# SamsungLabs/Metis

Measured on AMD Instinct MI355X. Metric: best_plan_iter_time_ms, lower is better.
Workload: dtype bf16; 1 GPU; model=gpt3-2.7b, global_batch=16, seq_len=2048, parallelism=dp1_tp1_pp1, microbatch=16

## Files before the change

### metis_amd/models/gpt.py

```python

from __future__ import annotations

import math
from dataclasses import dataclass
from typing import List, Optional

import torch
import torch.utils.checkpoint
import torch.distributed as dist
import torch.nn as nn
import torch.nn.functional as F

from metis_amd.ops import LayerNorm
from metis_amd.ops import residual as _res
from metis_amd.ops.attention import decode_attention, packed_flash_attention
from metis_amd.ops.cross_entropy import cross_entropy
from metis_amd.ops.mlp import fused_mlp
from metis_amd.ops.relayout import heads_merge, qkv_split_transpose
from metis_amd.partial_grads import mark_partial

import os as _os


@dataclass(frozen=True)
class GPTModelSpec:
    name: str
    hidden_size: int
    num_layers: int
    num_heads: int
    vocab_size: int
    seq_length: int
    ffn_hidden_size: Optional[int] = None
    num_kv_heads: Optional[int] = None

    @property
    def ffn(self) -> int:
        return self.ffn_hidden_size or 4 * self.hidden_size

    @property
# ... 193 lines not shown
        return _VocabParallelCrossEntropyBF16.apply(
            logits2d.contiguous(), labels, group)
    return _VocabParallelCrossEntropy.apply(
        logits2d.float().contiguous(), labels, group)


def _init_linear(weight: torch.Tensor, fan_in: int) -> None:
    std = 1.0 / math.sqrt(fan_in)
    nn.init.normal_(weight, mean=0.0, std=std)


class ColumnParallelLinear(nn.Module):

    def __init__(self, in_features: int, out_features: int, tp: int, dtype):
        super().__init__()
        assert out_features % tp == 0
        self.out_per_rank = out_features // tp
        self.weight = nn.Parameter(torch.empty(self.out_per_rank, in_features, dtype=dtype))
        self.bias = nn.Parameter(torch.zeros(self.out_per_rank, dtype=dtype))
        _init_linear(self.weight, in_features)

    def forward(self, x: torch.Tensor, tp_group) -> torch.Tensor:
        x = _CopyToTP.apply(x, tp_group)
        return F.linear(x, self.weight, self.bias)


class RowParallelLinear(nn.Module):

    def __init__(self, in_features: int, out_features: int, tp: int, dtype):
        super().__init__()
        assert in_features % tp == 0
        self.in_per_rank = in_features // tp
        self.weight = nn.Parameter(torch.empty(out_features, self.in_per_rank, dtype=dtype))
        self.bias = nn.Parameter(torch.zeros(out_features, dtype=dtype))
        _init_linear(self.weight, in_features)

    def forward(self, x: torch.Tensor, tp_group) -> torch.Tensor:
        y = F.linear(x, self.weight)
        y = _ReduceFromTP.apply(y, tp_group)
        return y + self.bias


class GPTBlock(nn.Module):
    def __init__(self, spec: GPTModelSpec, tp: int, dtype):
        super().__init__()
        h = spec.hidden_size
        assert spec.num_heads % tp == 0, "num_heads must divide by tp"
        self.heads_per_rank = spec.num_heads // tp
        self.head_dim = spec.head_dim

        self.ln_attn = LayerNorm(h)
        self.qkv = ColumnParallelLinear(h, 3 * h, tp, dtype)
        self.proj = RowParallelLinear(h, h, tp, dtype)
        self.ln_mlp = LayerNorm(h)
        self.fc1 = ColumnParallelLinear(h, spec.ffn, tp, dtype)
        self.fc2 = RowParallelLinear(spec.ffn, h, tp, dtype)
        self._lt_mlp = _os.environ.get("METIS_FC1_EPILOGUE") == "1"


    def _cached_attention(self, q, k, v, mask=None):
        new, total = q.size(2), k.size(2)
        if mask is not None:
            return F.scaled_dot_product_attention(q, k, v, attn_mask=mask)
        if new == 1:
            return decode_attention(q, k, v)
        mask = torch.ones(new, total, dtype=torch.bool, device=q.device)
        mask = torch.tril(mask, diagonal=total - new)
        return F.scaled_dot_product_attention(q, k, v, attn_mask=mask)

    def _forward_fused(self, x: torch.Tensor, tp_group) -> torch.Tensor:
        x, y = _res.norm_passthrough(
            x, self.ln_attn.weight, self.ln_attn.bias, self.ln_attn.eps)
        qkv = self.qkv(y, tp_group)
        attn = packed_flash_attention(
            qkv, self.heads_per_rank, self.heads_per_rank, self.head_dim
        )
        part = _ReduceFromTP.apply(F.linear(attn, self.proj.weight), tp_group)
        x, y = _res.bias_residual_layer_norm(
            part, self.proj.bias, x, self.ln_mlp.weight, self.ln_mlp.bias,
            self.ln_mlp.eps)
        h = F.linear(_CopyToTP.apply(y, tp_group), self.fc1.weight,
                     self.fc1.bias.detach())
        a = _res.gelu_bgrad(h, self.fc1.bias)
        part = _ReduceFromTP.apply(F.linear(a, self.fc2.weight), tp_group)
        return _res.bias_residual_add(part, self.fc2.bias, x)

    def forward(self, x: torch.Tensor, tp_group, sp: bool = False,
                cache=None, layer_idx: int = 0) -> torch.Tensor:
        if cache is not None:
            residual = x
            y = self.ln_attn(x)
            qkv = self.qkv(y, tp_group)
            q, k, v = qkv_split_transpose(
                qkv, self.heads_per_rank, self.heads_per_rank, self.head_dim)
            k, v = cache.append(layer_idx, k, v)
            if hasattr(cache, "kv_lens") and q.size(2) == 1:
                scales = getattr(cache, "kv_scales", None)
                scales = scales(layer_idx) if scales is not None else None
                if scales is None:
                    attn = decode_attention(q, k, v, kv_lens=cache.kv_lens())
                else:
                    attn = decode_attention(q, k, v, kv_lens=cache.kv_lens(),
                                            k_scale=scales[0],
                                            v_scale=scales[1])
            else:
                am = getattr(cache, "attention_mask", None)
                mask = am(k.size(2), q.device) if am is not None else None
# ... 177 lines not shown
```

### metis_amd/ops/adamw.py

```python

from __future__ import annotations

from typing import Iterable, List, Optional

import torch
import torch.distributed as dist

from metis_amd import ops as _ops


class FusedAdamW:
    def __init__(
        self,
        params: Iterable[torch.nn.Parameter],
        lr: float = 1e-4,
        betas=(0.9, 0.95),
        eps: float = 1e-8,
        weight_decay: float = 0.1,
        shard_group: Optional[object] = None,
    ) -> None:
        self.params: List[torch.nn.Parameter] = [p for p in params if p.requires_grad]
        if not self.params:
            raise ValueError("no trainable parameters")
        self.lr = lr
        self.beta1, self.beta2 = betas
        self.eps = eps
        self.weight_decay = weight_decay
        self.step_count = 0
        self.shard_group = shard_group
        ws = dist.get_world_size(shard_group) if shard_group is not None else 1
        self._shard_ws = ws
# ... 69 lines not shown
            self.m.mul_(self.beta1).add_(g, alpha=1 - self.beta1)
            self.v.mul_(self.beta2).addcmul_(g, g, value=1 - self.beta2)
            mhat = self.m / (1 - self.beta1 ** self.step_count)
            vhat = self.v / (1 - self.beta2 ** self.step_count)
            self.master.add_(
                -self.lr * (mhat / (vhat.sqrt() + self.eps)
                            + self.weight_decay * self.master)
            )

    def _gather_weight_shards(self) -> torch.Tensor:
        full = torch.empty(self._n, dtype=torch.float32,
                           device=self.master.device)
        try:
            dist.all_gather_into_tensor(full, self.master, group=self.shard_group)
        except (RuntimeError, ValueError):
            parts = [torch.empty_like(self.master) for _ in range(self._shard_ws)]
            dist.all_gather(parts, self.master, group=self.shard_group)
            full = torch.cat(parts)
        return full

    @torch.no_grad()
    def step(self, grad_scale: float = 1.0, pre_gathered: bool = False) -> None:
        self.step_count += 1
        grads = self._grad_flat if pre_gathered else self._gather_grads()

        if self._shard_ws > 1:
            off, n = self._shard_off, self._shard_n
            model = (self._model_flat[off:off + n]
                     if self._model_flat is not None else torch.Tensor())
            self._update(grads[off:off + n], model, grad_scale)
            if self._model_flat is not None:
                shard = self._model_flat[off:off + n].clone()
                dist.all_gather_into_tensor(self._model_flat, shard,
                                            group=self.shard_group)
                return
            full = self._gather_weight_shards()
            for p, (o, pn) in zip(self.params, self._slices):
                p.copy_(full[o:o + pn].view_as(p).to(p.dtype))
            return

        model = self._model_flat if self._model_flat is not None else torch.Tensor()
        self._update(grads, model, grad_scale)
        if self._model_flat is not None:
            return
        for p, (off, n) in zip(self.params, self._slices):
            p.copy_(self.master[off:off + n].view_as(p).to(p.dtype))

    def state_dict(self) -> dict:
        return {
            "step": self.step_count,
            "master": self.master,
            "m": self.m,
            "v": self.v,
        }

    def load_state_dict(self, state: dict) -> None:
        self.step_count = state["step"]
        self.master.copy_(state["master"])
        self.m.copy_(state["m"])
        self.v.copy_(state["v"])
```

### metis_amd/ops/hip/bindings.cpp

```cpp
#include <torch/extension.h>

#include <vector>

std::vector<torch::Tensor> layernorm_fwd(
    torch::Tensor x, torch::Tensor gamma, torch::Tensor beta, double eps);
std::vector<torch::Tensor> layernorm_bwd(
    torch::Tensor dy, torch::Tensor x, torch::Tensor gamma,
    torch::Tensor mean, torch::Tensor rstd);
std::vector<torch::Tensor> bias_residual_layernorm_fwd(
    torch::Tensor y, torch::Tensor bias, torch::Tensor residual,
    torch::Tensor gamma, torch::Tensor beta, double eps);
torch::Tensor bias_residual_add(
    torch::Tensor y, torch::Tensor bias, torch::Tensor residual);
std::vector<torch::Tensor> layernorm_bwd_add(
    torch::Tensor dy, torch::Tensor dres, torch::Tensor x, torch::Tensor gamma,
    torch::Tensor mean, torch::Tensor rstd, bool want_colsum);
std::vector<torch::Tensor> gelu_tanh_bwd_bgrad(torch::Tensor h, torch::Tensor da);
void adamw_step(
    torch::Tensor master, torch::Tensor model, torch::Tensor grad,
    torch::Tensor m, torch::Tensor v,
    double lr, double beta1, double beta2, double eps,
    double weight_decay, long step, double grad_scale);
torch::Tensor attn_decode(
    torch::Tensor q, torch::Tensor k, torch::Tensor v, double scale);
// ... 46 lines not shown
torch::Tensor mfma_tile_probe(torch::Tensor a, torch::Tensor b);
torch::Tensor gemm8_bf16(torch::Tensor x, torch::Tensor w);
std::vector<torch::Tensor> rmsnorm_fwd(
    torch::Tensor x, torch::Tensor gamma, double eps);
std::vector<torch::Tensor> rmsnorm_bwd(
    torch::Tensor dy, torch::Tensor x, torch::Tensor gamma, torch::Tensor rstd);
torch::Tensor rope_apply(
    torch::Tensor x, torch::Tensor cos_t, torch::Tensor sin_t, bool backward);
torch::Tensor swiglu_fwd(torch::Tensor a, torch::Tensor b);
std::vector<torch::Tensor> swiglu_bwd(
    torch::Tensor dy, torch::Tensor a, torch::Tensor b);
std::vector<torch::Tensor> cross_entropy_fwd(
    torch::Tensor logits, torch::Tensor labels);
torch::Tensor cross_entropy_bwd(
    torch::Tensor logits, torch::Tensor labels, torch::Tensor lse,
    torch::Tensor grad_scale);
std::vector<torch::Tensor> qkv_split_transpose(
    torch::Tensor qkv, long nq, long nkv, long head_dim);
torch::Tensor qkv_split_transpose_bwd(
    torch::Tensor dq, torch::Tensor dk, torch::Tensor dv, long head_dim);
torch::Tensor heads_merge(torch::Tensor x);
torch::Tensor heads_unmerge(torch::Tensor y, long H);
torch::Tensor tr16_probe(long stride_elems);

PYBIND11_MODULE(TORCH_EXTENSION_NAME, m) {
    m.def("layernorm_fwd", &layernorm_fwd,
          "fused LayerNorm forward (bf16, fp32 stats)");
    m.def("layernorm_bwd", &layernorm_bwd,
          "fused LayerNorm backward (dx + dgamma/dbeta)");
    m.def("bias_residual_layernorm_fwd", &bias_residual_layernorm_fwd,
          "x = residual + (y + bias) with both bf16 roundings, then "
          "LayerNorm(x) -> (x, z, mean, rstd)");
    m.def("bias_residual_add", &bias_residual_add,
          "x = residual + (y + bias) with both bf16 roundings");
    m.def("layernorm_bwd_add", &layernorm_bwd_add,
          "LayerNorm backward with a residual gradient folded in -> "
          "(g = dres + dx, dgamma, dbeta, colsum of g in fp32 or empty)");
    m.def("gelu_tanh_bwd_bgrad", &gelu_tanh_bwd_bgrad,
          "tanh-GeLU backward -> (dh bf16, dbias = column sums of dh, fp32)");
    m.def("adamw_step", &adamw_step, "fused AdamW step");
    m.def("attn_fwd", &attn_fwd,
          "flash attention forward (causal, GQA) -> (O, LSE)");
    m.def("attn_bwd", &attn_bwd,
          "flash attention backward -> (dQ, dK_per_head, dV_per_head)");
    m.def("attn_bwd_delta", &attn_bwd_delta,
          "rowsum(dO * O) in fp32 -> [B,H,S] (contiguous bf16 inputs)");
// ... 49 lines not shown
          pybind11::arg("v_scale"), pybind11::arg("slots"),
          pybind11::arg("pos"));
    m.def("w8_linear", &w8_linear,
          "fp8 (e4m3fn) weight-only linear for 1 <= M <= 16 bf16 rows: "
          "scale[n] * (x @ w8^T) + bias, fp32 accumulation, split-K",
          pybind11::arg("x"), pybind11::arg("w8"), pybind11::arg("scale"),
          pybind11::arg("bias") = pybind11::none(),
          pybind11::arg("num_splits") = 0);
    m.def("w8_linear_auto_splits", &w8_linear_auto_splits,
          "split count w8_linear picks for num_splits = 0 (from N and K only)");
    m.def("ce_row_max", &ce_row_max, "per-row max of bf16 logits (fp32)");
    m.def("ce_row_sumexp", &ce_row_sumexp,
          "per-row sum(exp(x - m)) of bf16 logits (fp32)");
    m.def("qkv_rope_split", &qkv_rope_split,
          "fused QKV relayout + RoPE (neox) forward");
    m.def("qkv_rope_split_bwd", &qkv_rope_split_bwd,
          "fused QKV relayout + RoPE backward gather");
    m.def("lt_fp8_matmul", &lt_fp8_matmul,
          "fp8 e4m3 GEMM with per-tensor scales, bf16 out");
    m.def("lt_fc1_forward", &lt_fc1_forward,
          "hipblaslt GEMM with GELU_AUX_BIAS epilogue (fc1 fused)");
    m.def("lt_matmul_dgelu_bgrad", &lt_matmul_dgelu_bgrad,
          "hipblaslt GEMM with DGELU_BGRAD epilogue (fc2 data grad fused)");
    m.def("tr16_probe", &tr16_probe,
          "ds_read_b64_tr_b16 lane-semantics probe (debug)");
}
```

### metis_amd/ops/hip/lt_gemm.cpp

```cpp

#include <torch/extension.h>

#include <hipblaslt/hipblaslt.h>

#include <c10/hip/HIPStream.h>

#include <mutex>
#include <stdexcept>
#include <string>
#include <unordered_map>

namespace {

#define LT_CHECK(expr)                                                        \
    do {                                                                      \
        hipblasStatus_t s_ = (expr);                                          \
        TORCH_CHECK(s_ == HIPBLAS_STATUS_SUCCESS, "hipblaslt error ",         \
                    (int)s_, " at ", #expr);                                  \
    } while (0)

hipblasLtHandle_t lt_handle() {
    static hipblasLtHandle_t handle = [] {
        hipblasLtHandle_t h;
        LT_CHECK(hipblasLtCreate(&h));
        return h;
    }();
    return handle;
}

constexpr size_t kWorkspaceBytes = 64ull << 20;

torch::Tensor workspace(const torch::TensorOptions& opt) {
    static torch::Tensor ws;
    if (!ws.defined() || ws.numel() < (long)kWorkspaceBytes)
        ws = torch::empty({(long)kWorkspaceBytes},
                          opt.dtype(torch::kUInt8));
    return ws;
}

struct LtPlan {
    hipblasLtMatmulDesc_t desc{};
    hipblasLtMatrixLayout_t a{}, b{}, d{};
    hipblasLtMatmulAlgo_t algo{};
    bool has_algo = false;
};

std::unordered_map<std::string, LtPlan>& plan_cache() {
    static std::unordered_map<std::string, LtPlan> cache;
    return cache;
}
std::mutex cache_mutex;

LtPlan& get_plan(hipblasLtEpilogue_t epi, bool transa, long M, long N, long K,
                 const void* bias, const void* aux, long aux_ld) {
    std::lock_guard<std::mutex> lock(cache_mutex);
    std::string key = std::to_string((int)epi) + (transa ? "t" : "n") + "_" +
                      std::to_string(M) + "_" + std::to_string(N) + "_" +
                      std::to_string(K);
    auto it = plan_cache().find(key);
    if (it != plan_cache().end()) return it->second;

    LtPlan plan;
    LT_CHECK(hipblasLtMatmulDescCreate(&plan.desc, HIPBLAS_COMPUTE_32F,
                                       HIP_R_32F));
    hipblasOperation_t opA = transa ? HIPBLAS_OP_T : HIPBLAS_OP_N;
    hipblasOperation_t opN = HIPBLAS_OP_N;
    LT_CHECK(hipblasLtMatmulDescSetAttribute(
        plan.desc, HIPBLASLT_MATMUL_DESC_TRANSA, &opA, sizeof(opA)));
    LT_CHECK(hipblasLtMatmulDescSetAttribute(
        plan.desc, HIPBLASLT_MATMUL_DESC_TRANSB, &opN, sizeof(opN)));
    LT_CHECK(hipblasLtMatmulDescSetAttribute(
        plan.desc, HIPBLASLT_MATMUL_DESC_EPILOGUE, &epi, sizeof(epi)));
    if (bias != nullptr)
        LT_CHECK(hipblasLtMatmulDescSetAttribute(
            plan.desc, HIPBLASLT_MATMUL_DESC_BIAS_POINTER, &bias,
            sizeof(bias)));
    if (aux != nullptr) {
        LT_CHECK(hipblasLtMatmulDescSetAttribute(
            plan.desc, HIPBLASLT_MATMUL_DESC_EPILOGUE_AUX_POINTER, &aux,
            sizeof(aux)));
        LT_CHECK(hipblasLtMatmulDescSetAttribute(
            plan.desc, HIPBLASLT_MATMUL_DESC_EPILOGUE_AUX_LD, &aux_ld,
            sizeof(aux_ld)));
    }

    if (transa)
        LT_CHECK(hipblasLtMatrixLayoutCreate(&plan.a, HIP_R_16BF, K, N, K));
    else
        LT_CHECK(hipblasLtMatrixLayoutCreate(&plan.a, HIP_R_16BF, N, K, N));
    LT_CHECK(hipblasLtMatrixLayoutCreate(&plan.b, HIP_R_16BF, K, M, K));
    LT_CHECK(hipblasLtMatrixLayoutCreate(&plan.d, HIP_R_16BF, N, M, N));

    hipblasLtMatmulPreference_t pref;
    LT_CHECK(hipblasLtMatmulPreferenceCreate(&pref));
    uint64_t ws_bytes = kWorkspaceBytes;
    LT_CHECK(hipblasLtMatmulPreferenceSetAttribute(
        pref, HIPBLASLT_MATMUL_PREF_MAX_WORKSPACE_BYTES, &ws_bytes,
        sizeof(ws_bytes)));
    hipblasLtMatmulHeuristicResult_t result{};
    int found = 0;
    LT_CHECK(hipblasLtMatmulAlgoGetHeuristic(
        lt_handle(), plan.desc, plan.a, plan.b, plan.d, plan.d, pref, 1,
        &result, &found));
    LT_CHECK(hipblasLtMatmulPreferenceDestroy(pref));
    TORCH_CHECK(found > 0, "hipblaslt: no algorithm for epilogue ", (int)epi,
                " at M=", M, " N=", N, " K=", K);
    plan.algo = result.algo;
    plan.has_algo = true;
    return plan_cache().emplace(key, plan).first->second;
}

void run_matmul(LtPlan& plan, const void* wA, const void* xB, void* outD,
                const void* bias, const void* aux, long aux_ld,
                hipblasLtEpilogue_t epi, long M, long N, long K,
                const torch::TensorOptions& opt) {
    if (bias != nullptr)
        LT_CHECK(hipblasLtMatmulDescSetAttribute(
            plan.desc, HIPBLASLT_MATMUL_DESC_BIAS_POINTER, &bias,
            sizeof(bias)));
    if (aux != nullptr) {
        LT_CHECK(hipblasLtMatmulDescSetAttribute(
            plan.desc, HIPBLASLT_MATMUL_DESC_EPILOGUE_AUX_POINTER, &aux,
            sizeof(aux)));
        LT_CHECK(hipblasLtMatmulDescSetAttribute(
            plan.desc, HIPBLASLT_MATMUL_DESC_EPILOGUE_AUX_LD, &aux_ld,
            sizeof(aux_ld)));
    }
    float alpha = 1.0f, beta = 0.0f;
    auto ws = workspace(opt);
    auto stream = c10::hip::getCurrentHIPStream().stream();
    LT_CHECK(hipblasLtMatmul(
        lt_handle(), plan.desc, &alpha, wA, plan.a, xB, plan.b, &beta, outD,
        plan.d, outD, plan.d, plan.has_algo ? &plan.algo : nullptr,
        ws.data_ptr(), kWorkspaceBytes, stream));
}

}

std::vector<torch::Tensor> lt_fc1_forward(torch::Tensor x, torch::Tensor w,
                                          torch::Tensor bias) {
    TORCH_CHECK(x.is_cuda() && x.dtype() == torch::kBFloat16);
    TORCH_CHECK(x.dim() == 2 && w.dim() == 2 && x.size(1) == w.size(1),
                "x [M,K], w [N,K]");
    auto xc = x.contiguous(), wc = w.contiguous(), bc = bias.contiguous();
    const long M = x.size(0), K = x.size(1), N = w.size(0);
    auto y = torch::empty({M, N}, x.options());
    auto aux = torch::empty({M, N}, x.options());

    auto& plan = get_plan(HIPBLASLT_EPILOGUE_GELU_AUX_BIAS, true, M, N, K,
                          bc.data_ptr(), aux.data_ptr(), N);
    run_matmul(plan, wc.data_ptr(), xc.data_ptr(), y.data_ptr(),
               bc.data_ptr(), aux.data_ptr(), N,
               HIPBLASLT_EPILOGUE_GELU_AUX_BIAS, M, N, K, x.options());
    return {y, aux};
}

std::vector<torch::Tensor> lt_matmul_dgelu_bgrad(torch::Tensor dy,
                                                 torch::Tensor w2,
                                                 torch::Tensor pre_gelu) {
    TORCH_CHECK(dy.is_cuda() && dy.dtype() == torch::kBFloat16);
    TORCH_CHECK(dy.dim() == 2 && w2.dim() == 2 && dy.size(1) == w2.size(0),
                "dy [M,H], w2 [H,N]");
    auto dyc = dy.contiguous(), w2c = w2.contiguous();
    auto auxc = pre_gelu.contiguous();
    const long M = dy.size(0), H = dy.size(1), N = w2.size(1);
    TORCH_CHECK(pre_gelu.size(0) == M && pre_gelu.size(1) == N);
    auto dpre = torch::empty({M, N}, dy.options());
    auto dbias = torch::empty({N}, dy.options());

    auto& plan = get_plan(HIPBLASLT_EPILOGUE_DGELU_BGRAD, false, M, N, H,
                          dbias.data_ptr(), auxc.data_ptr(), N);
    run_matmul(plan, w2c.data_ptr(), dyc.data_ptr(), dpre.data_ptr(),
               dbias.data_ptr(), auxc.data_ptr(), N,
               HIPBLASLT_EPILOGUE_DGELU_BGRAD, M, N, H, dy.options());
    return {dpre, dbias};
}

torch::Tensor lt_fp8_matmul(torch::Tensor x, torch::Tensor w,
                            torch::Tensor scale_x, torch::Tensor scale_w) {
    TORCH_CHECK(x.is_cuda() && x.dtype() == torch::kFloat8_e4m3fn);
    TORCH_CHECK(w.dtype() == torch::kFloat8_e4m3fn);
    TORCH_CHECK(x.dim() == 2 && w.dim() == 2 && x.size(1) == w.size(1));
    TORCH_CHECK(scale_x.dtype() == torch::kFloat32 && scale_x.numel() == 1);
    auto xc = x.contiguous(), wc = w.contiguous();
    const long M = x.size(0), K = x.size(1), N = w.size(0);
    auto y = torch::empty({M, N},
                          x.options().dtype(torch::kBFloat16));

    std::lock_guard<std::mutex> lock(cache_mutex);
    std::string key = "fp8_" + std::to_string(M) + "_" + std::to_string(N) +
                      "_" + std::to_string(K);
    auto it = plan_cache().find(key);
    if (it == plan_cache().end()) {
        LtPlan plan;
// ... 21 lines not shown
        LT_CHECK(hipblasLtMatmulPreferenceDestroy(pref));
        TORCH_CHECK(found > 0, "hipblaslt: no fp8 algorithm at M=", M,
                    " N=", N, " K=", K);
        plan.algo = result.algo;
        plan.has_algo = true;
        it = plan_cache().emplace(key, plan).first;
    }
    LtPlan& plan = it->second;
    const void* sa = scale_w.data_ptr();
    const void* sb = scale_x.data_ptr();
    LT_CHECK(hipblasLtMatmulDescSetAttribute(
        plan.desc, HIPBLASLT_MATMUL_DESC_A_SCALE_POINTER, &sa, sizeof(sa)));
    LT_CHECK(hipblasLtMatmulDescSetAttribute(
        plan.desc, HIPBLASLT_MATMUL_DESC_B_SCALE_POINTER, &sb, sizeof(sb)));
    float alpha = 1.0f, beta = 0.0f;
    auto ws = workspace(y.options());
    auto stream = c10::hip::getCurrentHIPStream().stream();
    LT_CHECK(hipblasLtMatmul(
        lt_handle(), plan.desc, &alpha, wc.data_ptr(), plan.a, xc.data_ptr(),
        plan.b, &beta, y.data_ptr(), plan.d, y.data_ptr(), plan.d,
        &plan.algo, ws.data_ptr(), kWorkspaceBytes, stream));
    return y;
}
```

### metis_amd/runtime/runner.py

```python

from __future__ import annotations

import os
import time
from typing import List, Optional, Tuple

import torch
import torch.distributed as dist

from metis_amd.models.gpt import GPTModel, GPTModelSpec
from metis_amd.models.llama import LlamaModel, LlamaModelSpec
from metis_amd.models.moe import MoEModel, MoEModelSpec
from metis_amd.ops import FusedAdamW
from metis_amd.planner.volume import uniform_layer_split
from metis_amd.runtime.clip import global_grad_norm, shard_flags
from metis_amd.runtime.comm import ParallelContext
from metis_amd.runtime.grad_sync import GradBucketSync
from metis_amd.partial_grads import defer_partial, sync_partial_grads
from metis_amd.runtime.trace import tracer_from_env


class PlanRunner:
    def __init__(
        self,
        spec: GPTModelSpec,
        ctx: ParallelContext,
        mbs: int,
        gbs: int,
        layer_partition: Optional[List[int]] = None,
        lr: float = 1e-4,
        dtype: torch.dtype = torch.bfloat16,
        schedule: str = "gpipe",
        recompute: bool = False,
        zero1: bool = False,
        sp: bool = False,
        vpp: int = 1,
# ... 459 lines not shown
                  "threshold)", flush=True)

    def save_checkpoint(self, path: str) -> None:
        torch.save({
            "model": self.model.state_dict(),
            "optimizer": self.optimizer.state_dict(),
            "plan": {"dp": self.ctx.dp, "tp": self.ctx.tp, "pp": self.ctx.pp,
                     "mbs": self.mbs, "gbs": self.gbs, "vpp": self.vpp,
                     "layer_partition": self.layer_partition},
            "rank": self.ctx.rank,
            "data_gen": (self._data_gen.get_state()
                         if self._data_gen is not None else None),
            "data_cursor": (self.data_loader.state()
                            if self.data_loader is not None else None),
        }, path)

    def load_checkpoint(self, path: str) -> None:
        state = torch.load(path, map_location="cpu", weights_only=True)
        plan = state["plan"]
        assert (plan["dp"], plan["tp"], plan["pp"]) == (
            self.ctx.dp, self.ctx.tp, self.ctx.pp
        ), "checkpoint plan does not match the running plan"
        self.model.load_state_dict(state["model"])
        if state.get("data_gen") is not None:
            dev = self.ctx.device or torch.device("cpu")
            self._data_gen = torch.Generator(device=dev)
            self._data_gen.set_state(state["data_gen"])
        if state.get("data_cursor") is not None and self.data_loader is not None:
            self.data_loader.load_state(int(state["data_cursor"]))
        opt_state = state["optimizer"]
        self.optimizer.load_state_dict({
            "step": opt_state["step"],
            "master": opt_state["master"].to(self.optimizer.master.device),
            "m": opt_state["m"].to(self.optimizer.m.device),
            "v": opt_state["v"].to(self.optimizer.v.device),
        })

    def timed_steps(self, steps: int, warmup: int) -> float:
        for _ in range(warmup):
            self.train_step()
        if dist.is_initialized():
            dist.barrier()
        if torch.cuda.is_available():
            torch.cuda.synchronize()
        t0 = time.perf_counter()
        for _ in range(steps):
# ... 8 lines not shown
```

### setup.py

```python

import os

from setuptools import setup

os.environ.setdefault("PYTORCH_ROCM_ARCH", "gfx950")

from torch.utils.cpp_extension import BuildExtension, CUDAExtension

ROOT = os.path.dirname(os.path.abspath(__file__))
HIP_DIR = os.path.join(ROOT, "metis_amd", "ops", "hip")

sources = [
    os.path.join(HIP_DIR, "bindings.cpp"),
    os.path.join(HIP_DIR, "layernorm.hip"),
    os.path.join(HIP_DIR, "gelu.hip"),
    os.path.join(HIP_DIR, "adamw.hip"),
    os.path.join(HIP_DIR, "attention.hip"),
    os.path.join(HIP_DIR, "attention_bwd.hip"),
    os.path.join(HIP_DIR, "gemm.hip"),
    os.path.join(HIP_DIR, "gemm8.hip"),
    os.path.join(HIP_DIR, "rmsnorm.hip"),
    os.path.join(HIP_DIR, "rope.hip"),
    os.path.join(HIP_DIR, "swiglu.hip"),
    os.path.join(HIP_DIR, "cross_entropy.hip"),
    os.path.join(HIP_DIR, "relayout.hip"),
    os.path.join(HIP_DIR, "qkv_rope.hip"),
    os.path.join(HIP_DIR, "decode.hip"),
    os.path.join(HIP_DIR, "decode_ragged.hip"),
    os.path.join(HIP_DIR, "decode_ragged_fp8.hip"),
    os.path.join(HIP_DIR, "kv_quant.hip"),
    os.path.join(HIP_DIR, "w8_linear.hip"),
    os.path.join(HIP_DIR, "lt_gemm.cpp"),
]
sources = [s for s in sources if os.path.exists(s)]

setup(
    name="metis_amd_hip_ops",
    ext_modules=[
        CUDAExtension(
            name="metis_amd._hip_ops",
            sources=sources,
            libraries=["hipblaslt"],
            extra_compile_args={
                "cxx": ["-O3", "-std=c++17"],
                "nvcc": ["-O3", "-std=c++17"],
            },
        )
    ],
    cmdclass={"build_ext": BuildExtension.with_options(no_python_abi_suffix=False)},
)
```

Measured before the change: 688.4 ms.

## Route linear backward GEMMs through tuned hipBLASLt algorithms from a table

Adds a custom autograd linear whose backward looks up per-shape routes (aten, hipBLASLt with a fixed solution index, or hipBLASLt TN with a cached transposed weight) in a JSON table tuned for MI355X. The goal is faster dgrad and wgrad GEMMs than the aten default heuristic. The transposed-weight cache is invalidated by an epoch that the optimizer step and checkpoint load bump. If the table is missing or was tuned for another hipBLASLt version, everything falls back to aten.

After: 674.1 ms, median of 6. 1.02x faster.

```diff
diff --git a/metis_amd/models/gpt.py b/metis_amd/models/gpt.py
--- a/metis_amd/models/gpt.py
+++ b/metis_amd/models/gpt.py
@@ -15,6 +15,7 @@
 from metis_amd.ops import residual as _res
 from metis_amd.ops.attention import decode_attention, packed_flash_attention
 from metis_amd.ops.cross_entropy import cross_entropy
+from metis_amd.ops.linear import linear
 from metis_amd.ops.mlp import fused_mlp
 from metis_amd.ops.relayout import heads_merge, qkv_split_transpose
 from metis_amd.partial_grads import mark_partial
@@ -254,7 +255,7 @@
 
     def forward(self, x: torch.Tensor, tp_group) -> torch.Tensor:
         x = _CopyToTP.apply(x, tp_group)
-        return F.linear(x, self.weight, self.bias)
+        return linear(x, self.weight, self.bias)
 
 
 class RowParallelLinear(nn.Module):
@@ -268,7 +269,7 @@
         _init_linear(self.weight, in_features)
 
     def forward(self, x: torch.Tensor, tp_group) -> torch.Tensor:
-        y = F.linear(x, self.weight)
+        y = linear(x, self.weight)
         y = _ReduceFromTP.apply(y, tp_group)
         return y + self.bias
 
@@ -307,14 +308,14 @@
         attn = packed_flash_attention(
             qkv, self.heads_per_rank, self.heads_per_rank, self.head_dim
         )
-        part = _ReduceFromTP.apply(F.linear(attn, self.proj.weight), tp_group)
+        part = _ReduceFromTP.apply(linear(attn, self.proj.weight), tp_group)
         x, y = _res.bias_residual_layer_norm(
             part, self.proj.bias, x, self.ln_mlp.weight, self.ln_mlp.bias,
             self.ln_mlp.eps)
-        h = F.linear(_CopyToTP.apply(y, tp_group), self.fc1.weight,
-                     self.fc1.bias.detach())
+        h = linear(_CopyToTP.apply(y, tp_group), self.fc1.weight,
+                   self.fc1.bias.detach())
         a = _res.gelu_bgrad(h, self.fc1.bias)
-        part = _ReduceFromTP.apply(F.linear(a, self.fc2.weight), tp_group)
+        part = _ReduceFromTP.apply(linear(a, self.fc2.weight), tp_group)
         return _res.bias_residual_add(part, self.fc2.bias, x)
 
     def forward(self, x: torch.Tensor, tp_group, sp: bool = False,
diff --git a/metis_amd/ops/adamw.py b/metis_amd/ops/adamw.py
--- a/metis_amd/ops/adamw.py
+++ b/metis_amd/ops/adamw.py
@@ -7,6 +7,7 @@
 import torch.distributed as dist
 
 from metis_amd import ops as _ops
+from metis_amd.ops import linear as _linear
 
 
 class FusedAdamW:
@@ -122,6 +123,7 @@
     @torch.no_grad()
     def step(self, grad_scale: float = 1.0, pre_gathered: bool = False) -> None:
         self.step_count += 1
+        _linear.bump_epoch()
         grads = self._grad_flat if pre_gathered else self._gather_grads()
 
         if self._shard_ws > 1:
@@ -155,6 +157,7 @@
         }
 
     def load_state_dict(self, state: dict) -> None:
+        _linear.bump_epoch()
         self.step_count = state["step"]
         self.master.copy_(state["master"])
         self.m.copy_(state["m"])
diff --git a/metis_amd/ops/hip/bindings.cpp b/metis_amd/ops/hip/bindings.cpp
--- a/metis_amd/ops/hip/bindings.cpp
+++ b/metis_amd/ops/hip/bindings.cpp
@@ -92,6 +92,16 @@
 torch::Tensor heads_merge(torch::Tensor x);
 torch::Tensor heads_unmerge(torch::Tensor y, long H);
 torch::Tensor tr16_probe(long stride_elems);
+torch::Tensor lt_linear_dgrad_tn(torch::Tensor dy, torch::Tensor wt);
+torch::Tensor lt_linear_dgrad(torch::Tensor dy, torch::Tensor w, long algo);
+torch::Tensor lt_linear_wgrad(torch::Tensor dy, torch::Tensor x, long algo);
+long lt_version();
+std::vector<long> lt_supported_algos(
+    const std::string& op, long M, long N, long K);
+long lt_heuristic_algo(const std::string& op, long M, long N, long K);
+long lt_wgrad_bgradb_algos(long M, long N, long K);
+torch::Tensor transpose_bf16(torch::Tensor w);
+void transpose_bf16_out(torch::Tensor w, torch::Tensor wt);
 
 PYBIND11_MODULE(TORCH_EXTENSION_NAME, m) {
     m.def("layernorm_fwd", &layernorm_fwd,
@@ -187,6 +197,22 @@
           "hipblaslt GEMM with GELU_AUX_BIAS epilogue (fc1 fused)");
     m.def("lt_matmul_dgelu_bgrad", &lt_matmul_dgelu_bgrad,
           "hipblaslt GEMM with DGELU_BGRAD epilogue (fc2 data grad fused)");
+    m.def("lt_linear_dgrad_tn", &lt_linear_dgrad_tn,
+          "dx [M,K] = dy [M,N] @ wt [K,N]^T (hipBLASLt TN route)");
+    m.def("lt_linear_dgrad", &lt_linear_dgrad,
+          "dx [M,K] = dy [M,N] @ w [N,K]; algo = solution index or -1");
+    m.def("lt_linear_wgrad", &lt_linear_wgrad,
+          "dw [N,K] = dy [M,N]^T @ x [M,K]; algo = solution index or -1");
+    m.def("lt_version", &lt_version, "hipblasLtGetVersion");
+    m.def("lt_supported_algos", &lt_supported_algos,
+          "supported solution indices for op (dgrad_tn|dgrad|wgrad) at M,N,K");
+    m.def("lt_heuristic_algo", &lt_heuristic_algo,
+          "solution index of the heuristic's first choice");
+    m.def("lt_wgrad_bgradb_algos", &lt_wgrad_bgradb_algos,
+          "number of weight-gradient algorithms with the BGRADB epilogue");
+    m.def("transpose_bf16", &transpose_bf16, "wt [C,R] = w [R,C]^T");
+    m.def("transpose_bf16_out", &transpose_bf16_out,
+          "transpose into an existing [C,R] buffer");
     m.def("tr16_probe", &tr16_probe,
           "ds_read_b64_tr_b16 lane-semantics probe (debug)");
 }
diff --git a/metis_amd/ops/hip/lt_gemm.cpp b/metis_amd/ops/hip/lt_gemm.cpp
--- a/metis_amd/ops/hip/lt_gemm.cpp
+++ b/metis_amd/ops/hip/lt_gemm.cpp
@@ -2,13 +2,16 @@
 #include <torch/extension.h>
 
 #include <hipblaslt/hipblaslt.h>
+#include <hipblaslt/hipblaslt-ext.hpp>
 
 #include <c10/hip/HIPStream.h>
 
+#include <climits>
 #include <mutex>
 #include <stdexcept>
 #include <string>
 #include <unordered_map>
+#include <vector>
 
 namespace {
 
@@ -51,12 +54,22 @@
 }
 std::mutex cache_mutex;
 
-LtPlan& get_plan(hipblasLtEpilogue_t epi, bool transa, long M, long N, long K,
-                 const void* bias, const void* aux, long aux_ld) {
+void destroy_plan(LtPlan& plan) {
+    if (plan.a) hipblasLtMatrixLayoutDestroy(plan.a);
+    if (plan.b) hipblasLtMatrixLayoutDestroy(plan.b);
+    if (plan.d) hipblasLtMatrixLayoutDestroy(plan.d);
+    if (plan.desc) hipblasLtMatmulDescDestroy(plan.desc);
+    plan = LtPlan{};
+}
+
+LtPlan& get_plan(hipblasLtEpilogue_t epi, bool transa, bool transb, long m,
+                 long n, long k, int algo_index, const void* bias,
+                 const void* aux, long aux_ld) {
     std::lock_guard<std::mutex> lock(cache_mutex);
-    std::string key = std::to_string((int)epi) + (transa ? "t" : "n") + "_" +
-                      std::to_string(M) + "_" + std::to_string(N) + "_" +
-                      std::to_string(K);
+    std::string key = std::to_string((int)epi) + (transa ? "t" : "n") +
+                      (transb ? "t" : "n") + "_" + std::to_string(m) + "_" +
+                      std::to_string(n) + "_" + std::to_string(k) + "_" +
+                      std::to_string(algo_index);
     auto it = plan_cache().find(key);
     if (it != plan_cache().end()) return it->second;
 
@@ -64,11 +77,11 @@
     LT_CHECK(hipblasLtMatmulDescCreate(&plan.desc, HIPBLAS_COMPUTE_32F,
                                        HIP_R_32F));
     hipblasOperation_t opA = transa ? HIPBLAS_OP_T : HIPBLAS_OP_N;
-    hipblasOperation_t opN = HIPBLAS_OP_N;
+    hipblasOperation_t opB = transb ? HIPBLAS_OP_T : HIPBLAS_OP_N;
     LT_CHECK(hipblasLtMatmulDescSetAttribute(
         plan.desc, HIPBLASLT_MATMUL_DESC_TRANSA, &opA, sizeof(opA)));
     LT_CHECK(hipblasLtMatmulDescSetAttribute(
-        plan.desc, HIPBLASLT_MATMUL_DESC_TRANSB, &opN, sizeof(opN)));
+        plan.desc, HIPBLASLT_MATMUL_DESC_TRANSB, &opB, sizeof(opB)));
     LT_CHECK(hipblasLtMatmulDescSetAttribute(
         plan.desc, HIPBLASLT_MATMUL_DESC_EPILOGUE, &epi, sizeof(epi)));
     if (bias != nullptr)
@@ -85,11 +98,39 @@
     }
 
     if (transa)
-        LT_CHECK(hipblasLtMatrixLayoutCreate(&plan.a, HIP_R_16BF, K, N, K));
+        LT_CHECK(hipblasLtMatrixLayoutCreate(&plan.a, HIP_R_16BF, k, m, k));
     else
-        LT_CHECK(hipblasLtMatrixLayoutCreate(&plan.a, HIP_R_16BF, N, K, N));
-    LT_CHECK(hipblasLtMatrixLayoutCreate(&plan.b, HIP_R_16BF, K, M, K));
-    LT_CHECK(hipblasLtMatrixLayoutCreate(&plan.d, HIP_R_16BF, N, M, N));
+        LT_CHECK(hipblasLtMatrixLayoutCreate(&plan.a, HIP_R_16BF, m, k, m));
+    if (transb)
+        LT_CHECK(hipblasLtMatrixLayoutCreate(&plan.b, HIP_R_16BF, n, k, n));
+    else
+        LT_CHECK(hipblasLtMatrixLayoutCreate(&plan.b, HIP_R_16BF, k, n, k));
+    LT_CHECK(hipblasLtMatrixLayoutCreate(&plan.d, HIP_R_16BF, m, n, m));
+
+    if (algo_index >= 0) {
+        std::vector<int> index{algo_index};
+        std::vector<hipblasLtMatmulHeuristicResult_t> results;
+        hipblasStatus_t st =
+            hipblaslt_ext::getAlgosFromIndex(lt_handle(), index, results);
+        float alpha = 1.0f, beta = 0.0f;
+        size_t ws_needed = 0;
+        if (st == HIPBLAS_STATUS_SUCCESS && !results.empty())
+            st = hipblaslt_ext::matmulIsAlgoSupported(
+                lt_handle(), plan.desc, &alpha, plan.a, plan.b, &beta, plan.d,
+                plan.d, results[0].algo, ws_needed);
+        else if (st == HIPBLAS_STATUS_SUCCESS)
+            st = HIPBLAS_STATUS_INVALID_VALUE;
+        if (st != HIPBLAS_STATUS_SUCCESS || ws_needed > kWorkspaceBytes) {
+            destroy_plan(plan);
+            TORCH_CHECK(false, "hipblaslt: algorithm index ", algo_index,
+                        " is not supported for op ", (transa ? "T" : "N"),
+                        (transb ? "T" : "N"), " m=", m, " n=", n, " k=", k,
+                        " (status ", (int)st, ", workspace ", ws_needed, ")");
+        }
+        plan.algo = results[0].algo;
+        plan.has_algo = true;
+        return plan_cache().emplace(key, plan).first->second;
+    }
 
     hipblasLtMatmulPreference_t pref;
     LT_CHECK(hipblasLtMatmulPreferenceCreate(&pref));
@@ -103,8 +144,9 @@
         lt_handle(), plan.desc, plan.a, plan.b, plan.d, plan.d, pref, 1,
         &result, &found));
     LT_CHECK(hipblasLtMatmulPreferenceDestroy(pref));
+    if (found <= 0) destroy_plan(plan);
     TORCH_CHECK(found > 0, "hipblaslt: no algorithm for epilogue ", (int)epi,
-                " at M=", M, " N=", N, " K=", K);
+                " at m=", m, " n=", n, " k=", k);
     plan.algo = result.algo;
     plan.has_algo = true;
     return plan_cache().emplace(key, plan).first->second;
@@ -147,8 +189,8 @@
     auto y = torch::empty({M, N}, x.options());
     auto aux = torch::empty({M, N}, x.options());
 
-    auto& plan = get_plan(HIPBLASLT_EPILOGUE_GELU_AUX_BIAS, true, M, N, K,
-                          bc.data_ptr(), aux.data_ptr(), N);
+    auto& plan = get_plan(HIPBLASLT_EPILOGUE_GELU_AUX_BIAS, true, false, N, M,
+                          K, -1, bc.data_ptr(), aux.data_ptr(), N);
     run_matmul(plan, wc.data_ptr(), xc.data_ptr(), y.data_ptr(),
                bc.data_ptr(), aux.data_ptr(), N,
                HIPBLASLT_EPILOGUE_GELU_AUX_BIAS, M, N, K, x.options());
@@ -168,8 +210,8 @@
     auto dpre = torch::empty({M, N}, dy.options());
     auto dbias = torch::empty({N}, dy.options());
 
-    auto& plan = get_plan(HIPBLASLT_EPILOGUE_DGELU_BGRAD, false, M, N, H,
-                          dbias.data_ptr(), auxc.data_ptr(), N);
+    auto& plan = get_plan(HIPBLASLT_EPILOGUE_DGELU_BGRAD, false, false, N, M,
+                          H, -1, dbias.data_ptr(), auxc.data_ptr(), N);
     run_matmul(plan, w2c.data_ptr(), dyc.data_ptr(), dpre.data_ptr(),
                dbias.data_ptr(), auxc.data_ptr(), N,
                HIPBLASLT_EPILOGUE_DGELU_BGRAD, M, N, H, dy.options());
@@ -237,3 +279,158 @@
         &plan.algo, ws.data_ptr(), kWorkspaceBytes, stream));
     return y;
 }
+
+namespace {
+
+enum class BwdOp { DgradTN, Dgrad, Wgrad };
+
+BwdOp parse_bwd_op(const std::string& op) {
+    if (op == "dgrad_tn") return BwdOp::DgradTN;
+    if (op == "dgrad") return BwdOp::Dgrad;
+    if (op == "wgrad") return BwdOp::Wgrad;
+    TORCH_CHECK(false, "unknown op '", op, "' (dgrad_tn, dgrad, wgrad)");
+}
+
+struct BwdProblem {
+    bool transa, transb;
+    long m, n, k;
+};
+
+BwdProblem bwd_problem(BwdOp op, long M, long N, long K) {
+    switch (op) {
+    case BwdOp::DgradTN: return {true, false, K, M, N};
+    case BwdOp::Dgrad:   return {false, false, K, M, N};
+    default:             return {false, true, K, N, M};
+    }
+}
+
+void check_operand(const torch::Tensor& t, const char* name) {
+    TORCH_CHECK(t.is_cuda(), name, " must be a CUDA tensor");
+    TORCH_CHECK(t.dtype() == torch::kBFloat16, name, " must be bf16");
+    TORCH_CHECK(t.dim() == 2, name, " must be 2-d");
+    TORCH_CHECK(t.is_contiguous(), name, " must be contiguous");
+    TORCH_CHECK(t.numel() > 0, name, " must not be empty");
+    TORCH_CHECK(reinterpret_cast<uintptr_t>(t.data_ptr()) % 16 == 0, name,
+                " must be 16-byte aligned");
+}
+
+void check_pair(const torch::Tensor& a, const char* an,
+                const torch::Tensor& b, const char* bn) {
+    check_operand(a, an);
+    check_operand(b, bn);
+    TORCH_CHECK(a.device() == b.device(), an, " and ", bn,
+                " must be on one device");
+}
+
+torch::Tensor run_bwd(BwdOp op, long M, long N, long K, long algo,
+                      const torch::Tensor& colA, const torch::Tensor& colB,
+                      long out_rows, long out_cols) {
+    TORCH_CHECK(algo >= -1 && algo <= INT_MAX, "bad algorithm index ", algo);
+    BwdProblem p = bwd_problem(op, M, N, K);
+    auto& plan = get_plan(HIPBLASLT_EPILOGUE_DEFAULT, p.transa, p.transb, p.m,
+                          p.n, p.k, (int)algo, nullptr, nullptr, 0);
+    auto out = torch::empty({out_rows, out_cols}, colA.options());
+    run_matmul(plan, colA.data_ptr(), colB.data_ptr(), out.data_ptr(), nullptr,
+               nullptr, 0, HIPBLASLT_EPILOGUE_DEFAULT, M, N, K,
+               colA.options());
+    return out;
+}
+
+}
+
+torch::Tensor lt_linear_dgrad_tn(torch::Tensor dy, torch::Tensor wt) {
+    check_pair(dy, "dy", wt, "wt");
+    TORCH_CHECK(dy.size(1) == wt.size(1), "dy [M,N], wt [K,N]: inner sizes ",
+                dy.size(1), " and ", wt.size(1), " differ");
+    const long M = dy.size(0), N = dy.size(1), K = wt.size(0);
+    return run_bwd(BwdOp::DgradTN, M, N, K, -1, wt, dy, M, K);
+}
+
+torch::Tensor lt_linear_dgrad(torch::Tensor dy, torch::Tensor w, long algo) {
+    check_pair(dy, "dy", w, "w");
+    TORCH_CHECK(dy.size(1) == w.size(0), "dy [M,N], w [N,K]: inner sizes ",
+                dy.size(1), " and ", w.size(0), " differ");
+    const long M = dy.size(0), N = dy.size(1), K = w.size(1);
+    return run_bwd(BwdOp::Dgrad, M, N, K, algo, w, dy, M, K);
+}
+
+torch::Tensor lt_linear_wgrad(torch::Tensor dy, torch::Tensor x, long algo) {
+    check_pair(dy, "dy", x, "x");
+    TORCH_CHECK(dy.size(0) == x.size(0), "dy [M,N], x [M,K]: inner sizes ",
+                dy.size(0), " and ", x.size(0), " differ");
+    const long M = dy.size(0), N = dy.size(1), K = x.size(1);
+    return run_bwd(BwdOp::Wgrad, M, N, K, algo, x, dy, N, K);
+}
+
+
+long lt_version() {
+    int v = 0;
+    LT_CHECK(hipblasLtGetVersion(lt_handle(), &v));
+    return v;
+}
+
+std::vector<long> lt_supported_algos(const std::string& op, long M, long N,
+                                     long K) {
+    BwdProblem p = bwd_problem(parse_bwd_op(op), M, N, K);
+    std::vector<hipblasLtMatmulHeuristicResult_t> all;
+    LT_CHECK(hipblaslt_ext::getAllAlgos(
+        lt_handle(), hipblaslt_ext::GemmType::HIPBLASLT_GEMM,
+        p.transa ? HIPBLAS_OP_T : HIPBLAS_OP_N,
+        p.transb ? HIPBLAS_OP_T : HIPBLAS_OP_N, HIP_R_16BF, HIP_R_16BF,
+        HIP_R_16BF, HIP_R_16BF, HIPBLAS_COMPUTE_32F, all));
+    LtPlan* plan;
+    {
+        plan = &get_plan(HIPBLASLT_EPILOGUE_DEFAULT, p.transa, p.transb, p.m,
+                         p.n, p.k, -1, nullptr, nullptr, 0);
+    }
+    std::vector<long> out;
+    float alpha = 1.0f, beta = 0.0f;
+    for (auto& r : all) {
+        size_t ws_needed = 0;
+        hipblasStatus_t st = hipblaslt_ext::matmulIsAlgoSupported(
+            lt_handle(), plan->desc, &alpha, plan->a, plan->b, &beta, plan->d,
+            plan->d, r.algo, ws_needed);
+        if (st == HIPBLAS_STATUS_SUCCESS && ws_needed <= kWorkspaceBytes)
+            out.push_back(hipblaslt_ext::getIndexFromAlgo(r.algo));
+    }
+    return out;
+}
+
+long lt_heuristic_algo(const std::string& op, long M, long N, long K) {
+    BwdProblem p = bwd_problem(parse_bwd_op(op), M, N, K);
+    auto& plan = get_plan(HIPBLASLT_EPILOGUE_DEFAULT, p.transa, p.transb, p.m,
+                          p.n, p.k, -1, nullptr, nullptr, 0);
+    return hipblaslt_ext::getIndexFromAlgo(plan.algo);
+}
+
+long lt_wgrad_bgradb_algos(long M, long N, long K) {
+    BwdProblem p = bwd_problem(BwdOp::Wgrad, M, N, K);
+    LtPlan plan;
+    LT_CHECK(hipblasLtMatmulDescCreate(&plan.desc, HIPBLAS_COMPUTE_32F,
+                                       HIP_R_32F));
+    hipblasOperation_t opA = HIPBLAS_OP_N, opB = HIPBLAS_OP_T;
+    hipblasLtEpilogue_t epi = HIPBLASLT_EPILOGUE_BGRADB;
+    LT_CHECK(hipblasLtMatmulDescSetAttribute(
+        plan.desc, HIPBLASLT_MATMUL_DESC_TRANSA, &opA, sizeof(opA)));
+    LT_CHECK(hipblasLtMatmulDescSetAttribute(
+        plan.desc, HIPBLASLT_MATMUL_DESC_TRANSB, &opB, sizeof(opB)));
+    LT_CHECK(hipblasLtMatmulDescSetAttribute(
+        plan.desc, HIPBLASLT_MATMUL_DESC_EPILOGUE, &epi, sizeof(epi)));
+    LT_CHECK(hipblasLtMatrixLayoutCreate(&plan.a, HIP_R_16BF, p.m, p.k, p.m));
+    LT_CHECK(hipblasLtMatrixLayoutCreate(&plan.b, HIP_R_16BF, p.n, p.k, p.n));
+    LT_CHECK(hipblasLtMatrixLayoutCreate(&plan.d, HIP_R_16BF, p.m, p.n, p.m));
+    hipblasLtMatmulPreference_t pref;
+    LT_CHECK(hipblasLtMatmulPreferenceCreate(&pref));
+    uint64_t ws_bytes = kWorkspaceBytes;
+    LT_CHECK(hipblasLtMatmulPreferenceSetAttribute(
+        pref, HIPBLASLT_MATMUL_PREF_MAX_WORKSPACE_BYTES, &ws_bytes,
+        sizeof(ws_bytes)));
+    hipblasLtMatmulHeuristicResult_t results[8];
+    int found = 0;
+    hipblasStatus_t st = hipblasLtMatmulAlgoGetHeuristic(
+        lt_handle(), plan.desc, plan.a, plan.b, plan.d, plan.d, pref, 8,
+        results, &found);
+    hipblasLtMatmulPreferenceDestroy(pref);
+    destroy_plan(plan);
+    return st == HIPBLAS_STATUS_SUCCESS ? found : 0;
+}
diff --git a/metis_amd/ops/hip/transpose.hip b/metis_amd/ops/hip/transpose.hip
--- /dev/null
+++ b/metis_amd/ops/hip/transpose.hip
@@ -0,0 +1,93 @@
+
+#include <torch/extension.h>
+#include <c10/hip/HIPStream.h>
+
+#include "common.h"
+
+namespace {
+
+constexpr int TR_TILE = 64;
+constexpr int TR_BLOCK = 256;
+constexpr int TR_PITCH = TR_TILE + 8;
+constexpr int TR_GROUP_SHIFT = 8;
+constexpr int TR_LDS_ELEMS =
+    TR_TILE * TR_PITCH + (TR_TILE / 8) * TR_GROUP_SHIFT;
+constexpr int TR_CHUNKS = TR_TILE * TR_TILE / 8;
+
+__device__ __forceinline__ int tr_lds_offset(int r, int c) {
+    return r * TR_PITCH + (r >> 3) * TR_GROUP_SHIFT + c;
+}
+
+__global__ __launch_bounds__(TR_BLOCK) void transpose_bf16_kernel(
+    const short* __restrict__ in, short* __restrict__ out, int R, int C,
+    int tiles_c) {
+    __shared__ __attribute__((aligned(16))) short tile[TR_LDS_ELEMS];
+
+    const int tile_r = blockIdx.x / tiles_c;
+    const int tile_c = blockIdx.x - tile_r * tiles_c;
+    const long r_base = (long)tile_r * TR_TILE;
+    const long c_base = (long)tile_c * TR_TILE;
+
+    #pragma unroll
+    for (int chunk = threadIdx.x; chunk < TR_CHUNKS; chunk += TR_BLOCK) {
+        const int r = chunk >> 3, k = chunk & 7;
+        const long gr = r_base + r, gc = c_base + k * 8;
+        bf16x8 v = {0, 0, 0, 0, 0, 0, 0, 0};
+        if (gr < R && gc < C)
+            v = *reinterpret_cast<const bf16x8*>(in + gr * C + gc);
+        *reinterpret_cast<bf16x8*>(&tile[tr_lds_offset(r, k * 8)]) = v;
+    }
+    __syncthreads();
+
+    #pragma unroll
+    for (int chunk = threadIdx.x; chunk < TR_CHUNKS; chunk += TR_BLOCK) {
+        const int c = chunk >> 3, i = chunk & 7;
+        const long gc = c_base + c, gr0 = r_base + i * 8;
+        if (gc < C && gr0 < R) {
+            bf16x8 v;
+            #pragma unroll
+            for (int j = 0; j < 8; ++j) v[j] = tile[tr_lds_offset(i * 8 + j, c)];
+            *reinterpret_cast<bf16x8*>(out + gc * R + gr0) = v;
+        }
+    }
+}
+
+void check_matrix(const torch::Tensor& t, const char* name) {
+    TORCH_CHECK(t.is_cuda(), name, " must be a CUDA tensor");
+    TORCH_CHECK(t.dtype() == torch::kBFloat16, name, " must be bf16");
+    TORCH_CHECK(t.dim() == 2, name, " must be 2-d");
+    TORCH_CHECK(t.is_contiguous(), name, " must be contiguous");
+    TORCH_CHECK(reinterpret_cast<uintptr_t>(t.data_ptr()) % 16 == 0, name,
+                " must be 16-byte aligned");
+}
+
+}
+
+void transpose_bf16_out(torch::Tensor w, torch::Tensor wt) {
+    check_matrix(w, "w");
+    check_matrix(wt, "wt");
+    const long R = w.size(0), C = w.size(1);
+    TORCH_CHECK(R > 0 && C > 0 && R % 8 == 0 && C % 8 == 0,
+                "transpose_bf16: both sizes must be positive multiples of 8, "
+                "got [", R, ", ", C, "]");
+    TORCH_CHECK(wt.size(0) == C && wt.size(1) == R, "wt must be [", C, ", ", R,
+                "]");
+    TORCH_CHECK(w.device() == wt.device(), "w and wt must be on one device");
+    TORCH_CHECK(w.data_ptr() != wt.data_ptr(), "w and wt must not alias");
+    const long tiles_r = (R + TR_TILE - 1) / TR_TILE;
+    const long tiles_c = (C + TR_TILE - 1) / TR_TILE;
+    TORCH_CHECK(R <= INT_MAX && C <= INT_MAX && tiles_r * tiles_c <= INT_MAX,
+                "transpose_bf16: matrix too large");
+    hipLaunchKernelGGL(transpose_bf16_kernel, dim3((unsigned)(tiles_r * tiles_c)),
+        dim3(TR_BLOCK), 0, c10::hip::getCurrentHIPStream().stream(),
+        reinterpret_cast<const short*>(w.data_ptr()),
+        reinterpret_cast<short*>(wt.data_ptr()), (int)R, (int)C, (int)tiles_c);
+    HIP_CHECK_LAST();
+}
+
+torch::Tensor transpose_bf16(torch::Tensor w) {
+    check_matrix(w, "w");
+    auto wt = torch::empty({w.size(1), w.size(0)}, w.options());
+    transpose_bf16_out(w, wt);
+    return wt;
+}
diff --git a/metis_amd/ops/linear.py b/metis_amd/ops/linear.py
--- /dev/null
+++ b/metis_amd/ops/linear.py
@@ -0,0 +1,228 @@
+
+from __future__ import annotations
+
+import json
+import logging
+import os
+from typing import Dict, Optional, Tuple
+
+import torch
+import torch.nn.functional as F
+
+from metis_amd import ops as _ops
+
+_log = logging.getLogger(__name__)
+
+TABLE_PATH = os.path.join(
+    os.path.dirname(os.path.dirname(os.path.dirname(os.path.abspath(__file__)))),
+    "profiles", "mi355x", "gemm_algos.json")
+
+OPS = ("dgrad", "wgrad")
+ROUTES = {"dgrad": ("aten", "lt", "lt_tn"), "wgrad": ("aten", "lt")}
+
+Key = Tuple[str, int, int, int]
+
+
+class GemmTable:
+
+    def __init__(self, lt_version: int, device: str,
+                 entries: Dict[Key, Tuple[str, int]]):
+        self.lt_version = lt_version
+        self.device = device
+        self.entries = entries
+
+    @classmethod
+    def empty(cls) -> "GemmTable":
+        return cls(-1, "", {})
+
+    @classmethod
+    def parse(cls, obj) -> "GemmTable":
+        if not isinstance(obj, dict):
+            raise ValueError("table is not an object")
+        version, device = obj.get("hipblaslt_version"), obj.get("device")
+        if not _is_int(version) or not isinstance(device, str):
+            raise ValueError("header needs hipblaslt_version (int) and device")
+        raw = obj.get("entries")
+        if not isinstance(raw, list):
+            raise ValueError("entries is not a list")
+        entries: Dict[Key, Tuple[str, int]] = {}
+        for e in raw:
+            if not isinstance(e, dict):
+                raise ValueError("entry is not an object")
+            op, route, algo = e.get("op"), e.get("route"), e.get("algo", -1)
+            dims = (e.get("M"), e.get("N"), e.get("K"))
+            if op not in OPS or route not in ROUTES[op]:
+                raise ValueError(f"bad op/route {op!r}/{route!r}")
+            if not all(_is_int(d) and d > 0 for d in dims):
+                raise ValueError(f"bad shape {dims!r}")
+            if not _is_int(algo) or algo < -1:
+                raise ValueError(f"bad algo {algo!r}")
+            key = (op,) + dims
+            if key in entries:
+                raise ValueError(f"duplicate entry {key!r}")
+            entries[key] = (route, algo)
+        return cls(version, device, entries)
+
+    def matches(self, lt_version: int, device: str) -> bool:
+        return self.lt_version == lt_version and self.device == device
+
+    def lookup(self, op: str, M: int, N: int, K: int) -> Tuple[str, int]:
+        return self.entries.get((op, M, N, K), ("aten", -1))
+
+
+def _is_int(v) -> bool:
+    return isinstance(v, int) and not isinstance(v, bool)
+
+
+def load_table(path: str) -> GemmTable:
+    try:
+        with open(path) as f:
+            return GemmTable.parse(json.load(f))
+    except (OSError, ValueError) as e:
+        _log.warning("gemm table %s not used (%s): linear backward GEMMs "
+                     "take the aten route", path, e)
+        return GemmTable.empty()
+
+
+def resolve_table(table: GemmTable, lt_version: int, device: str) -> GemmTable:
+    if not table.entries or table.matches(lt_version, device):
+        return table
+    _log.warning(
+        "gemm table was tuned for hipBLASLt %s on %r, this is %s on %r: "
+        "linear backward GEMMs take the aten route",
+        table.lt_version, table.device, lt_version, device)
+    return GemmTable.empty()
+
+
+_FILE_TABLE = load_table(os.environ.get("METIS_GEMM_TABLE") or TABLE_PATH)
+_ACTIVE: Optional[GemmTable] = None
+
+
+def device_id() -> str:
+    p = torch.cuda.get_device_properties(torch.cuda.current_device())
+    return f"{p.gcnArchName.split(':')[0]}-{p.multi_processor_count}cu"
+
+
+def _active_table() -> GemmTable:
+    global _ACTIVE
+    if _ACTIVE is None:
+        ext = _ops.require_extension()
+        _ACTIVE = resolve_table(_FILE_TABLE, int(ext.lt_version()),
+                                device_id())
+    return _ACTIVE
+
+
+class use_table:
+
+    def __init__(self, table: GemmTable):
+        self.table = table
+
+    def __enter__(self):
+        global _ACTIVE
+        self._saved = _ACTIVE
+        _ACTIVE = self.table
+        return self.table
+
+    def __exit__(self, *exc):
+        global _ACTIVE
+        _ACTIVE = self._saved
+        return False
+
+
+def enabled() -> bool:
+    return os.environ.get("METIS_LT_BWD", "1") != "0"
+
+
+_epoch = 0
+transpose_refreshes = 0
+
+
+def bump_epoch() -> None:
+    global _epoch
+    _epoch += 1
+
+
+def _stamp(weight: torch.Tensor):
+    return (_epoch, weight._version, weight.data_ptr(),
+            getattr(weight, "_metis_fwd_count", 0))
+
+
+def transposed_weight(weight: torch.Tensor) -> torch.Tensor:
+    global transpose_refreshes
+    ext = _ops.require_extension()
+    stamp = _stamp(weight)
+    cached = getattr(weight, "_metis_wt", None)
+    if cached is not None and cached[0] == stamp:
+        return cached[1]
+    w = weight.detach()
+    if (cached is not None and cached[1].device == w.device
+            and cached[1].shape == (w.size(1), w.size(0))):
+        wt = cached[1]
+    else:
+        wt = torch.empty(w.size(1), w.size(0), dtype=w.dtype, device=w.device)
+    ext.transpose_bf16_out(w, wt)
+    weight._metis_wt = (stamp, wt)
+    transpose_refreshes += 1
+    return wt
+
+
+def _lt_ok(*tensors: torch.Tensor) -> bool:
+    if not all(t.is_cuda and t.dtype == torch.bfloat16 for t in tensors):
+        return False
+    return not torch.cuda.is_current_stream_capturing()
+
+
+def _lt_operand(t: torch.Tensor) -> torch.Tensor:
+    t = t.contiguous()
+    return t if t.data_ptr() % 16 == 0 else t.clone()
+
+
+class _Linear(torch.autograd.Function):
+    @staticmethod
+    def forward(ctx, x, weight, bias):
+        ctx.save_for_backward(x, weight)
+        ctx.has_bias = bias is not None
+        weight._metis_fwd_count = getattr(weight, "_metis_fwd_count", 0) + 1
+        ctx.weight_ref = weight
+        return F.linear(x, weight, bias)
+
+    @staticmethod
+    def backward(ctx, dy):
+        x, w = ctx.saved_tensors
+        N, K = w.shape
+        dy2 = dy.reshape(-1, N)
+        x2 = x.reshape(-1, K)
+        M = dy2.size(0)
+        lt = _lt_ok(dy2, x2, w)
+        table = _active_table() if lt else None
+        dx = dw = db = None
+
+        if ctx.needs_input_grad[0]:
+            route, algo = table.lookup("dgrad", M, N, K) if lt else ("aten", -1)
+            if route == "lt_tn" and N % 8 == 0 and K % 8 == 0:
+                wt = transposed_weight(ctx.weight_ref)
+                dx2 = _ops.require_extension().lt_linear_dgrad_tn(
+                    _lt_operand(dy2), wt)
+            elif route == "lt":
+                dx2 = _ops.require_extension().lt_linear_dgrad(
+                    _lt_operand(dy2), _lt_operand(w), algo)
+            else:
+                dx2 = dy2 @ w
+            dx = dx2.view(x.shape)
+        if ctx.needs_input_grad[1]:
+            route, algo = table.lookup("wgrad", M, N, K) if lt else ("aten", -1)
+            if route == "lt":
+                dw = _ops.require_extension().lt_linear_wgrad(
+                    _lt_operand(dy2), _lt_operand(x2), algo)
+            else:
+                dw = dy2.t() @ x2
+        if ctx.has_bias and ctx.needs_input_grad[2]:
+            db = dy2.sum(0, keepdim=True).view(N)
+        return dx, dw, db
+
+
+def linear(x: torch.Tensor, weight: torch.Tensor,
+           bias: Optional[torch.Tensor] = None) -> torch.Tensor:
+    if not enabled():
+        return F.linear(x, weight, bias)
+    return _Linear.apply(x, weight, bias)
diff --git a/metis_amd/runtime/runner.py b/metis_amd/runtime/runner.py
--- a/metis_amd/runtime/runner.py
+++ b/metis_amd/runtime/runner.py
@@ -12,6 +12,7 @@
 from metis_amd.models.llama import LlamaModel, LlamaModelSpec
 from metis_amd.models.moe import MoEModel, MoEModelSpec
 from metis_amd.ops import FusedAdamW
+from metis_amd.ops.linear import bump_epoch
 from metis_amd.planner.volume import uniform_layer_split
 from metis_amd.runtime.clip import global_grad_norm, shard_flags
 from metis_amd.runtime.comm import ParallelContext
@@ -517,6 +518,7 @@
             self.ctx.dp, self.ctx.tp, self.ctx.pp
         ), "checkpoint plan does not match the running plan"
         self.model.load_state_dict(state["model"])
+        bump_epoch()
         if state.get("data_gen") is not None:
             dev = self.ctx.device or torch.device("cpu")
             self._data_gen = torch.Generator(device=dev)
diff --git a/setup.py b/setup.py
--- a/setup.py
+++ b/setup.py
@@ -31,6 +31,7 @@
     os.path.join(HIP_DIR, "kv_quant.hip"),
     os.path.join(HIP_DIR, "w8_linear.hip"),
     os.path.join(HIP_DIR, "lt_gemm.cpp"),
+    os.path.join(HIP_DIR, "transpose.hip"),
 ]
 sources = [s for s in sources if os.path.exists(s)]
 
```
